# imironhead/ml_super_resolution

Measured on AMD Instinct MI355X. Metric: VDSR-20 training patches/sec (41x41, batch 256 per GPU); fwd HR megapixels/sec alongside, higher is better.
Workload: dtype f32; 1 GPU; BASELINE configs[2]: VDSR 20-layer 3x3x64 residual, RGB, batch 256x41x41 per GPU, fwd+bwd+TF-Adam, random-init weights; global_batch=256, patch=41, parallelism=dp1

## Files before the change

### ml_super_resolution_amd/csrc/conv_chain.hip

```cpp
#include "launchers.h"
namespace srx {

template <bool WT, int AUX>
__global__ __launch_bounds__(256, 1) void conv_chain_kernel(const ConvArgs a, const ChainPtrs c) {
    for (int l = 0; l < c.L; ++l) {
        ConvArgs al = a;
        al.x = c.x[l]; al.w = c.w[l]; al.bias = c.bias[l]; al.y = c.y[l];
        if (WT) al.mask = c.aux[l];
        else al.skip = c.aux[l];
        asm volatile("" : "+s"(al.N), "+s"(al.H), "+s"(al.W), "+s"(al.OH), "+s"(al.OW), "+s"(al.Cin), "+s"(al.Cout));
        asm volatile("" : "+s"(al.pad_t), "+s"(al.pad_l), "+s"(al.TH), "+s"(al.TW), "+s"(al.NTX), "+s"(al.RS));
        asm volatile("" : "+s"(al.units_total), "+s"(al.act), "+s"(al.post_relu), "+s"(al.mask_act), "+s"(al.buf_floats));
        conv_pipe_body<3, 3, 64, 4, WT, AUX, false>(al, l == 0);
        asm volatile("s_waitcnt vmcnt(0)" ::: "memory");
        __builtin_amdgcn_fence(__ATOMIC_RELEASE, "workgroup");
        __builtin_amdgcn_s_barrier();
        __builtin_amdgcn_fence(__ATOMIC_ACQUIRE, "workgroup");
    }
}

hipError_t launch_conv_chain(bool wt, bool aux, const ConvArgs& a, const ChainPtrs& c, int grid, size_t lds, hipStream_t s) {
    if (!wt) return aux ? hipErrorInvalidValue : launch_chain_with_lds(conv_chain_kernel<false, 0>, a, c, grid, lds, s);
    return aux ? launch_chain_with_lds(conv_chain_kernel<true, 1>, a, c, grid, lds, s)
               : launch_chain_with_lds(conv_chain_kernel<true, 0>, a, c, grid, lds, s);
}
}
```

### ml_super_resolution_amd/csrc/conv_kernels.hip.h

```cpp
#pragma once
#include <hip/hip_runtime.h>
#include <stdint.h>
#include <type_traits>

namespace srx {

typedef float f32x4 __attribute__((ext_vector_type(4)));

enum { ACT_NONE = 0, ACT_RELU = 1, ACT_TANH = 2, ACT_LRELU = 3, ACT_SIGMOID = 4 };

struct ConvArgs {
    const float* x;
    const float* w;
    const float* bias;
    const float* skip;
    const float* mask;
    float* y;
    int N, H, W, OH, OW, Cin, Cout;
    int pad_t, pad_l;
    int TH, TW, NTX, RS;
    int units_total;
    int act, post_relu, mask_act;
    float inv_rs;
    int stagger;
    int dbg;
    unsigned long long* trace;
    int buf_floats;
    int stride;
    int d2s_r, d2s_rc;
};

struct WgradArgs {
    const float* x;
    const float* dpre;
    float* part;
    int part_stride;
    int N, H, W, OH, OW, Cin, Cout;
    int pad_t, pad_l;
    int TH, TW, NTX, RS;
    int units_total;
    float inv_rs;
    int stagger;
    int zero_slot;
    int stride;
    unsigned long long* trace;
};

constexpr int kChainMax = 32;
struct ChainPtrs {
    const float* x[kChainMax];
    const float* w[kChainMax];
    const float* bias[kChainMax];
    const float* aux[kChainMax];
    float* y[kChainMax];
    int L;
};

template <int CINP>
struct Lds {
    static constexpr int PS = (CINP == 4) ? 4 : CINP + 4;
};

__device__ __forceinline__ float srx_tanhf(float x) {
    const float ax = fabsf(x);
    const float x2 = ax * ax;
    float p = fmaf(x2, -0.006274174898862839f, 0.021071631461381912f);
    p = fmaf(x2, p, -0.053852297365665436f);
    p = fmaf(x2, p, 0.13332585990428925f);
    p = fmaf(x2, p, -0.33333316445350647f);
    const float small = fmaf(x2 * ax, p, ax);
    const float e = __builtin_amdgcn_exp2f(ax * 2.8853900817779268f);
    const float big = fmaf(-2.0f, __builtin_amdgcn_rcpf(e + 1.0f), 1.0f);
    return copysignf(ax < 0.55f ? small : big, x);
}

typedef float f32x2 __attribute__((ext_vector_type(2)));
__device__ __forceinline__ f32x2 srx_tanhf2(f32x2 x) {
    const f32x2 ax = {fabsf(x[0]), fabsf(x[1])};
    const f32x2 x2 = ax * ax;
    f32x2 p = __builtin_elementwise_fma(x2, f32x2{-0.006274174898862839f, -0.006274174898862839f}, f32x2{0.021071631461381912f, 0.021071631461381912f});
    p = __builtin_elementwise_fma(x2, p, f32x2{-0.053852297365665436f, -0.053852297365665436f});
    p = __builtin_elementwise_fma(x2, p, f32x2{0.13332585990428925f, 0.13332585990428925f});
    p = __builtin_elementwise_fma(x2, p, f32x2{-0.33333316445350647f, -0.33333316445350647f});
    const f32x2 small = __builtin_elementwise_fma(x2 * ax, p, ax);
    const f32x2 t = ax * 2.8853900817779268f;
    f32x2 e = {__builtin_amdgcn_exp2f(t[0]), __builtin_amdgcn_exp2f(t[1])};
    e = e + 1.0f;
    const f32x2 r = {__builtin_amdgcn_rcpf(e[0]), __builtin_amdgcn_rcpf(e[1])};
// ... 319 lines not shown
#pragma unroll
            for (int tap = 0; tap < TAPS; ++tap)
#pragma unroll
                for (int j = 0; j < KSPT; ++j) {
                    const int soff = ((tap * a.Cin + 16 * (j / 4) + (j % 4)) * a.Cout) * 4;
                    wr[tap * KSPT + j] = __builtin_bit_cast(float, __builtin_amdgcn_raw_buffer_load_b32(rsrc, vlane, soff, 0));
                }
        } else {
            const int vlane = (co * a.Cin + 4 * kq) * 4;
#pragma unroll
            for (int tap = 0; tap < TAPS; ++tap)
#pragma unroll
                for (int g = 0; g < KSPT / 4; ++g) {
                    const int soff = (((TAPS - 1 - tap) * a.Cout) * a.Cin + 16 * g) * 4;
                    const f32x4 v = __builtin_bit_cast(f32x4, __builtin_amdgcn_raw_buffer_load_b128(rsrc, vlane, soff, 0));
#pragma unroll
                    for (int e = 0; e < 4; ++e) wr[tap * KSPT + 4 * g + e] = v[e];
                }
        }
        return;
    }
    const bool co_ok = co < a.Cout;
#pragma unroll
    for (int tap = 0; tap < TAPS; ++tap) {
#pragma unroll
        for (int j = 0; j < KSPT; ++j) {
            const int ci = (CINP >= 16) ? 16 * (j / 4) + 4 * kq + (j % 4) : kq;
            const bool ok = co_ok & (ci < a.Cin);
            const unsigned idx = !WT ? (unsigned)((tap * a.Cin + ci) * a.Cout + co)
                                     : (unsigned)(((TAPS - 1 - tap) * a.Cout + co) * a.Cin + ci);
            const float v = a.w[ok ? idx : 0u];
            wr[tap * KSPT + j] = ok ? v : 0.f;
        }
    }
}

template <int KH, int KW, int CINP, int G, bool GUARD, bool AUX>
__device__ __forceinline__ void conv_group(const float* lds, const float (&wr)[KH * KW * (CINP / 4)],
                                           const f32x4 bias4, const ConvArgs& a, int n, int h, int ow0,
                                           int th, int tw, float inv_tw, int m_first, int m_step, int n_active,
                                           int li, int kq, int cout0, unsigned long long& t_mfma, unsigned long long& t_pro,
                                           unsigned long long& t_epi) {
    constexpr int PS = Lds<CINP>::PS;
    constexpr int NG = (CINP >= 16) ? CINP / 16 : 1;
    const unsigned long long ts_pro = SRX_STAMP();
    const int npx = th * tw;
    const int cb = cout0 + 4 * kq;
    const bool vec = ((a.Cout & 3) == 0) && (cb + 3 < a.Cout) && !a.d2s_r;
    const size_t img_base = (size_t)n * a.OH * a.OW * a.Cout;
    int laddr[G];
    unsigned off[G];
    bool valid[G];
    f32x4 acc[G];
#pragma unroll
    for (int i = 0; i < G; ++i) {
        const int t = 16 * (m_first + i * m_step) + li;
        const bool live = (t < npx) & (i < n_active);
        valid[i] = live & (cb < a.Cout);
        const int tt = live ? t : 0;
        const int orow = fdiv_small(tt, inv_tw, tw);
        const int ocol = tt - orow * tw;
        laddr[i] = ((orow * a.RS + ocol) * PS << (a.stride - 1)) + ((CINP >= 16) ? 4 * kq : kq);
        off[i] = !valid[i] ? 0u
                 : (a.d2s_r ? (unsigned)(((h + orow) * a.d2s_r * a.OW + ow0 + ocol) * a.d2s_rc)
                            : (unsigned)(((h + orow) * a.OW + ow0 + ocol) * a.Cout + cb));
        acc[i] = bias4;
// ... 293 lines not shown
}

template <int CINP, int NB, bool Z = false, bool MID = false>
__device__ __forceinline__ void stage_tile_scalar(StageSeq& qi, StageSeq& qc, const StageGeo& G, __amdgpu_buffer_rsrc_t rsrc,
                                                  int voff_lane, int wl_lane) {
    constexpr int PPP = 256 / (CINP / 4);
    while (qi.left > 0) {
        f32x4 v[NB];
        unsigned long long mk[NB];
#pragma unroll
        for (int i = 0; i < NB; ++i) {
            unsigned long long t;
            int so;
            if constexpr (Z) {
                unsigned long long m;
                stage_mask_az<MID>(qi, G, m, t, mk[i]);
                stage_mask_bz(qi, m, t, mk[i], so);
                v[i] = stage_fire_z(m, mk[i], so, rsrc, voff_lane);
            } else {
                stage_mask_a(qi, G, mk[i], t);
                stage_mask_b(qi, mk[i], t, so);
                v[i] = stage_fire(mk[i], so, rsrc, voff_lane);
            }
            stage_next<PPP * CINP * 4>(qi, G.JP1, G.rowfix_g);
        }
#pragma unroll
        for (int i = 0; i < NB; ++i) {
            stage_commit((Z ? 2 : 1) * (NB - 1 - i), qc, mk[i], wl_lane, v[i]);
            stage_next<PPP * Lds<CINP>::PS * 4>(qc, G.JP1, G.rowfix_l);
        }
    }
}

#define SRX_PIN(x) asm volatile("" : "+v"(x))

template <int MAXG, int AUX>
struct PipePend {
    f32x4 acc[MAXG];
    f32x4 aux[(AUX == 1 || AUX == 2) ? MAXG : 1];
    __amdgpu_buffer_rsrc_t yrs;
    int m_first, gs;
};
struct PipeEpi {
    int lo, lo2;
    int cout4;
    int sh, rowb;
    int vo1, vo2, vo3;
};
template <int AUX>
__device__ __forceinline__ PipeEpi pipe_epi_setup(const ConvArgs& a) {
    PipeEpi e;
    e.lo = (a.act == ACT_RELU) ? 0 : (int)0x80000000;
    e.lo2 = (AUX == 2 && a.post_relu) ? 0 : (int)0x80000000;
    e.cout4 = (AUX == 4) ? 3 * a.d2s_r * 4 : a.Cout * 4;
    e.sh = (a.TW >= 32) ? 1 : 0;
    e.rowb = (AUX == 4) ? a.d2s_r * (a.OW * a.d2s_r * 3) * 4 : a.OW * a.Cout * 4;
    e.vo1 = e.vo2 = e.vo3 = 0;
    return e;
}
__device__ __forceinline__ f32x4 clamp_lo4(f32x4 v, int lo) {
#pragma unroll
    for (int e = 0; e < 4; ++e) {
        const float f = v[e];
        const int b = __float_as_int(f);
        v[e] = __int_as_float(b > lo ? b : lo);
    }
// ... 147 lines not shown
                for (int i = 2; i < nfr; ++i) frag(i);
                if (t < NST) {
                    if constexpr (Z) stg[t] = stage_fire_z(mv, mr, so, xrs, voff_lane);
                    else stg[t] = stage_fire(mk[t], so, xrs, voff_lane);
                }
                if (t >= NBLK / 2 && t < NBLK / 2 + NST) stage_next<PPP * PS * 4>(qc, SG.JP1, SG.rowfix_l);
            } else {
                if (t < NST) stage_next<PPP * CINP * 4>(qi, SG.JP1, SG.rowfix_g);
                if (t == A0) {
                    tcur += gs * TSTEP;
#pragma unroll
                    for (int i = 0; i < MAXG; ++i) lan[i] = *reinterpret_cast<const int*>(ldsb + tcur + i * TSTEP);
                }
            }
        }
#pragma unroll
        for (int i = 0; i < nfr; ++i) cg[i] = nxt[i];
    }
#pragma unroll
    for (int i = 0; i < MAXG; ++i) { cur[i] = cg[i]; la[i] = lan[i]; }
    if constexpr (G == 4)
        asm volatile("s_nop 15\n\ts_nop 7" : "+v"(acc[0]), "+v"(acc[1]), "+v"(acc[2]), "+v"(acc[3]));
    else
        asm volatile("s_nop 15\n\ts_nop 7" : "+v"(acc[0]), "+v"(acc[1]), "+v"(acc[2]));
#pragma unroll
    for (int i = 0; i < MAXG; ++i) {
        pd.acc[i] = (i < G) ? acc[i < G ? i : 0] : bias4;
        if (HASAUX) pd.aux[i] = (i < G) ? aux[i < G ? i : 0] : bias4;
    }
    pd.yrs = un.yrs; pd.m_first = m_first; pd.gs = gs;
    tt[1] += SRX_STAMP() - ts_m;
}

template <int KH, int KW, int CINP, int NCH, bool WT, int AUX, bool Z>
__device__ __forceinline__ void conv_pipe_body(const ConvArgs& a, bool lds_setup = true) {
    extern __shared__ __attribute__((aligned(16))) float lds[];
    constexpr int TAPS = KH * KW;
    constexpr int KSPT = CINP / 4;
    constexpr int NPART = 4 / NCH;
    constexpr int TPP = CINP / 4, PPP = 256 / TPP;
    constexpr int PS = Lds<CINP>::PS;
    constexpr int MAXG = 4;
    constexpr int TSTEP = 16 * PS * 4 * NPART;
    const int tid = threadIdx.x;
    const int lane = tid & 63;
    const int wave = __builtin_amdgcn_readfirstlane(tid >> 6);
    const int li = lane & 15, kq = lane >> 4;
    const int chunk = wave % NCH, part = wave / NCH;
    const int cout0 = chunk * 16;
    const int cb = cout0 + 4 * kq;
    const int c4 = tid % TPP, sp = tid / TPP;
    char* ldsb = reinterpret_cast<char*>(lds);

#ifdef SRX_TRACE
    const unsigned long long t_entry = __builtin_amdgcn_s_memtime(), rt_entry = __builtin_amdgcn_s_memrealtime();
#endif
    float wr[TAPS * KSPT];
    load_stationary_weights<TAPS, CINP, WT>(wr, a, cout0, li, kq);
    f32x4 bias4 = {0.f, 0.f, 0.f, 0.f};
    if (a.bias) {
#pragma unroll
        for (int e = 0; e < 4; ++e)
            if (cb + e < a.Cout) bias4[e] = a.bias[cb + e];
    }

    const long G_ = gridDim.x;
    const int u0 = (int)(((long)blockIdx.x * a.units_total) / G_);
    const int u1 = (int)(((long)(blockIdx.x + 1) * a.units_total) / G_);
    if (u0 >= u1) return;
    const int buf_bytes = a.buf_floats * 4;
    const int rows_full = a.TH + KH - 1;
    const int row_stride_b = a.RS * PS * 4;

    if (lds_setup) {
        const f32x4 z = {0.f, 0.f, 0.f, 0.f};
        for (int i = tid; !Z && i < (rows_full + 1) * a.pad_l * TPP; i += 256) {
            const int q = i / TPP, ch = i % TPP;
            const int r = q / a.pad_l, c = q % a.pad_l;
            const int off = ((r * a.RS + c) * PS + 4 * ch) * 4;
            if ((r * a.RS + c) * PS * 4 < buf_bytes) {
                *reinterpret_cast<f32x4*>(ldsb + off) = z;
                *reinterpret_cast<f32x4*>(ldsb + buf_bytes + off) = z;
            }
        }
        const int tw_ = Z ? a.TW : a.OW;
        const int n_sub_max = (a.TH * tw_ + 15) >> 4;
        for (int i = tid; i < n_sub_max * 64; i += 256) {
            const int m = i >> 6, L = i & 63;
            const int t = 16 * m + (L & 15);
            int addr = 0;
            if (t < a.TH * tw_) {
                const int orow = t / tw_, ocol = t - orow * tw_;
                addr = ((orow * a.RS + ocol) * PS + 4 * (L >> 4)) * 4;
            }
            const int where = ((16 * m + (L >> 2)) * PS + CINP + (L & 3)) * 4;
            *reinterpret_cast<int*>(ldsb + where) = addr;
// ... 29 lines not shown
        h = u % a.OH;
        n = u / a.OH;
        ow0 = 0;
        if constexpr (Z) {
            const int tx = n % a.NTX;
            n = n / a.NTX;
            ow0 = tx * a.TW;
            if (ow0 > a.OW - a.TW) ow0 = a.OW - a.TW;
        }
        th = a.TH;
        if (a.OH - h < th) th = a.OH - h;
        if (u1 - u < th) th = u1 - u;
    };
    auto stage_setup = [&](StageSeq& qi, StageSeq& qc, int h, int th, int ow0, int buf, bool active) {
        const int left = __builtin_amdgcn_readfirstlane(active ? (th + KH - 1) * JP : 0);
        qi.j = 0; qc.j = 0;
        qi.off = __builtin_amdgcn_readfirstlane(((h - a.pad_t) * a.W + ow0) * CINP * 4);
        if constexpr (Z) {
            SG.m_first = uniform64(__ballot(ow0 - a.pad_l + sp >= 0));
            const int c = (JP - 1) * PPP + sp;
            SG.m_last = uniform64(__ballot(c < a.RS && ow0 - a.pad_l + c < a.W));
        }
        qc.off = __builtin_amdgcn_readfirstlane(buf * buf_bytes);
        qi.left = left; qc.left = left;
        const int above = (a.pad_t > h) ? (a.pad_t - h) * JP : 0;
        qi.thr = __builtin_amdgcn_readfirstlane(left - above);
        qc.thr = 0;
    };

    unsigned long long tt[4] = {0, 0, 0, 0};
    int n, h, th, ow0;
    tile_of(u0, n, h, th, ow0);
    [[maybe_unused]] const unsigned long long t_begin = SRX_STAMP();
    __syncthreads();
    {
        StageSeq qi, qc;
        stage_setup(qi, qc, h, th, ow0, 0, true);
        const __amdgpu_buffer_rsrc_t xrs = __builtin_amdgcn_make_buffer_rsrc(
            const_cast<float*>(a.x) + ((size_t)n * a.H * a.W - a.pad_l) * CINP, 0, (a.H * a.W + a.pad_l) * CINP * 4, 0x00020000);
        stage_tile_scalar<CINP, 6, Z>(qi, qc, SG, xrs, voff_lane, wl_lane);
    }
    lds_barrier();
#pragma unroll
    for (int i = 0; i < TAPS * KSPT; ++i) {
        float t = wr[i];
        asm volatile("v_accvgpr_write_b32 %0, %1" : "=a"(wr[i]) : "v"(t));
    }
    [[maybe_unused]] const unsigned long long t_first = SRX_STAMP();

    PipePend<MAXG, AUX> pd;
#pragma unroll
    for (int i = 0; i < MAXG; ++i) pd.acc[i] = bias4;
    if (AUX == 1 || AUX == 2) {
#pragma unroll
        for (int i = 0; i < MAXG; ++i) pd.aux[i] = bias4;
    }
    pd.yrs = __builtin_amdgcn_make_buffer_rsrc(a.y, 0, 0, 0x00020000); pd.m_first = 0; pd.gs = 0;

    int cur_buf = 0;
    int u = u0;
    while (u < u1) {
        const unsigned long long ts_u = SRX_STAMP();
        tile_of(u, n, h, th, ow0);
        const int un_ = u + th;
        const bool has_next = un_ < u1;
        int n2 = n, h2 = h, th2 = th, ow2 = ow0;
        if (has_next) tile_of(un_, n2, h2, th2, ow2);
        StageSeq qi, qc;
        stage_setup(qi, qc, h2, th2, ow2, cur_buf ^ 1, has_next);
        const __amdgpu_buffer_rsrc_t xrs = __builtin_amdgcn_make_buffer_rsrc(
            const_cast<float*>(a.x) + ((size_t)n2 * a.H * a.W - a.pad_l) * CINP, 0, (a.H * a.W + a.pad_l) * CINP * 4, 0x00020000);

        PipeUnit un;
        const int npx = th * (Z ? a.TW : a.OW);
        const size_t unit_off = (AUX == 4) ? (((size_t)n * a.OH + h) * a.d2s_r * a.OW + ow0) * (size_t)(3 * a.d2s_r)
                                           : (((size_t)n * a.OH + h) * a.OW + ow0) * a.Cout;
        const int unit_bytes = (AUX == 4) ? ((th * a.d2s_r - 1) * a.OW + a.TW) * ep.cout4
                                          : (Z ? (th - 1) * a.OW + a.TW : npx) * ep.cout4;
        un.yrs = __builtin_amdgcn_make_buffer_rsrc(a.y + unit_off, 0, unit_bytes, 0x00020000);
        un.auxrs = __builtin_amdgcn_make_buffer_rsrc(const_cast<float*>((AUX == 1 || AUX == 2) ? auxp + unit_off : a.x), 0,
                                                     (AUX == 1 || AUX == 2) ? unit_bytes : 0, 0x00020000);

        const int n_sub = (npx + 15) >> 4;
        const int cnt = (n_sub - part + NPART - 1) / NPART;
        if (cnt > 0) {
            const int ng = (cnt + MAXG - 1) / MAXG;
            const int base = cnt / ng, rem = cnt % ng;
            int tcur = cur_buf * buf_bytes + tlane;
            int la[MAXG];
#pragma unroll
            for (int i = 0; i < MAXG; ++i) la[i] = *reinterpret_cast<const int*>(ldsb + tcur + i * TSTEP);
            f32x4 cur[MAXG];
#pragma unroll
            for (int i = 0; i < MAXG; ++i) cur[i] = *reinterpret_cast<const f32x4*>(ldsb + la[i]);
            tt[0] += SRX_STAMP() - ts_u;
            int idx = 0;
            for (int gi = 0; gi < ng; ++gi) {
                const int gs = base + (gi < rem ? 1 : 0);
                const int m_first = part + idx * NPART;
                if (gs == MAXG)
                    conv_group_pipe<KH, KW, CINP, MAXG, MAXG, AUX, NPART, Z>(ldsb, wr, bias4, row_stride_b, qi, qc, SG, xrs, voff_lane,
                                                                          wl_lane, la, cur, tcur, pd, un, m_first, gs, ep, vst, tt);
                else
                    conv_group_pipe<KH, KW, CINP, MAXG - 1, MAXG, AUX, NPART, Z>(ldsb, wr, bias4, row_stride_b, qi, qc, SG, xrs, voff_lane,
                                                                              wl_lane, la, cur, tcur, pd, un, m_first, gs, ep, vst, tt);
                idx += gs;
            }
        }
        const unsigned long long ts_d = SRX_STAMP();
        stage_tile_scalar<CINP, 6, Z>(qi, qc, SG, xrs, voff_lane, wl_lane);
        lds_barrier();
        tt[3] += SRX_STAMP() - ts_d;
        cur_buf ^= 1;
        u = un_;
    }
#pragma unroll
    for (int i = 0; i < MAXG; ++i) pipe_epilogue_one<MAXG, AUX, NPART, Z>(pd, i, ep, vst);
#ifdef SRX_TRACE
    if (a.trace && lane == 0) {
        unsigned long long* tr = a.trace + ((size_t)blockIdx.x * 4 + wave) * 12;
        tr[0] = t_begin; tr[1] = SRX_STAMP(); tr[2] = tt[1]; tr[3] = tt[3];
        tr[4] = __builtin_amdgcn_s_getreg((15 << 11) | (0 << 6) | 4);
        tr[5] = rt_entry; tr[6] = __builtin_amdgcn_s_memrealtime(); tr[7] = t_entry;
        tr[8] = t_first - t_begin; tr[9] = 0; tr[10] = tt[0]; tr[11] = tt[2];
    }
#endif
}

template <int KH, int KW, int CINP, int NCH, bool WT, int AUX>
__global__ __launch_bounds__(256, 1) void conv_pipe_kernel(const ConvArgs a) {
    conv_pipe_body<KH, KW, CINP, NCH, WT, AUX, false>(a);
}
template <int KH, int KW, int CINP, int NCH, bool WT, int AUX>
__global__ __launch_bounds__(256, 1) void conv_pipe_strip_kernel(const ConvArgs a) {
    static_assert(NCH == 4 || NCH == 2, "strip tiles: 64 or 32 output channels");
    static_assert(AUX != 4 || (!WT && NCH == 2), "sub-pixel store: forward, <= 32 output channels");
    conv_pipe_body<KH, KW, CINP, NCH, WT, AUX, true>(a);
}

template <int CINP, bool WT, int G>
__device__ __forceinline__ void conv_group_generic(const float* lds, const f32x4 bias4, const ConvArgs& a, int KH,
                                                   int KW, int n, int h, int ow0, int th, int tw, float inv_tw,
                                                   int m_first, int m_step, int li, int kq, int cout0) {
    constexpr int PS = Lds<CINP>::PS;
    constexpr int NG = (CINP >= 16) ? CINP / 16 : 1;
    const int TAPS = KH * KW;
    const int npx = th * tw;
    const int cb = cout0 + 4 * kq;
    const bool vec = ((a.Cout & 3) == 0) && (cb + 3 < a.Cout) && !a.d2s_r;
    const size_t img_base = (size_t)n * a.OH * a.OW * a.Cout;
    int laddr[G];
    unsigned off[G];
    bool valid[G];
    f32x4 acc[G];
#pragma unroll
    for (int i = 0; i < G; ++i) {
        const int t = 16 * (m_first + i * m_step) + li;
        valid[i] = (t < npx) & (cb < a.Cout);
        const int tt = (t < npx) ? t : 0;
        const int orow = fdiv_small(tt, inv_tw, tw);
        const int ocol = tt - orow * tw;
        laddr[i] = ((orow * a.RS + ocol) * PS << (a.stride - 1)) + ((CINP >= 16) ? 4 * kq : kq);
        off[i] = !valid[i] ? 0u
                 : (a.d2s_r ? (unsigned)(((h + orow) * a.d2s_r * a.OW + ow0 + ocol) * a.d2s_rc)
// ... 1497 lines not shown
```

### ml_super_resolution_amd/csrc/srx_api.hip

```cpp
#include <math.h>
#include <stdarg.h>
#include <atomic>
#include <stdio.h>
#include <stdlib.h>
#include <string.h>

#include "../../include/srx.h"
#include "elementwise.h"
#include "launchers.h"
#include "bf16x3.h"

using namespace srx;

namespace {

thread_local char g_err[512] = "";

struct Knobs {
    int pipe_default, narrow, wgrad_lin, wgrad_pipe, wgrad_pipe_strip, wgrad_rows_full, wgrad_1x1, wgrad_pack3, kwrows_min_pixels, big_route_min_pixels, strip_d2s, conv_1x1_min_pixels, pack3_dgrad;
    int chain, wgrad_batch;
    unsigned long long* trace;
    int dbg;
};
int env_int(const char* name, int dflt) { const char* e = getenv(name); return e ? atoi(e) : dflt; }
// ... 359 lines not shown
    a->inv_rs = 1.0f / (float)p.RS;
    a->stride = 1;
    a->stagger = stagger_sleeps(p);
    a->dbg = knobs().dbg;
    a->trace = knobs().trace;
}

int chain_plan(const srx_conv_desc* d, int op, int in_act, Plan* p, ConvArgs* a, int* grid) {
    int rc = check_desc(d);
    if (rc) return rc;
    if (op != SRX_OP_FWD && op != SRX_OP_BWD_DATA) return fail(SRX_ERR_BAD_ARG, "chain: op %d (forward or data gradient)", op);
    if (!use_chain()) return fail(SRX_ERR_UNSUPPORTED, "chain: switched off (srx_set_chain / SRX_CHAIN)");
    if (!use_pipe()) return fail(SRX_ERR_UNSUPPORTED, "chain: conv path 0");
    if (!launch_conv_chain) return fail(SRX_ERR_UNSUPPORTED, "chain: this build has no chain kernels");
    if (d->precision != SRX_PRECISION_FP32) return fail(SRX_ERR_UNSUPPORTED, "chain: precision %d (exact fp32 only)", d->precision);
    if (d->KH != 3 || d->KW != 3 || d->Cin != 64 || d->Cout != 64 || d->stride != 1 || d->pad_mode != SRX_PAD_SAME)
        return fail(SRX_ERR_UNSUPPORTED, "chain: only 3x3 64->64 stride-1 SAME layers");
    if (d->subpixel_r > 1 || d->post_add_relu) return fail(SRX_ERR_UNSUPPORTED, "chain: no sub-pixel store or post-add activation");
    if (op == SRX_OP_FWD && d->act != SRX_ACT_NONE && d->act != SRX_ACT_RELU)
        return fail(SRX_ERR_UNSUPPORTED, "chain: forward activation %d (none / ReLU)", d->act);
    if (op == SRX_OP_BWD_DATA && in_act != SRX_ACT_NONE && in_act != SRX_ACT_RELU)
        return fail(SRX_ERR_UNSUPPORTED, "chain: in_act %d (none / ReLU)", in_act);
    int pt, pl, OH, OW;
    geometry(d, &pt, &pl, &OH, &OW);
    rc = (op == SRX_OP_FWD) ? make_plan(d->N, d->H, d->W, OH, OW, d->Cin, d->Cout, 3, 3, pt, pl, p, true)
                            : make_plan(d->N, OH, OW, d->H, d->W, d->Cout, d->Cin, 3, 3, 2 - pt, 2 - pl, p);
    if (rc) return rc;
    memset(a, 0, sizeof(*a));
    if (op == SRX_OP_FWD) fill_conv_args(a, *p, d->N, d->H, d->W, d->Cin, d->Cout);
    else fill_conv_args(a, *p, d->N, OH, OW, d->Cout, d->Cin);
    a->act = (op == SRX_OP_FWD) ? d->act : SRX_ACT_NONE;
    a->post_relu = 0;
    a->mask_act = (op == SRX_OP_FWD) ? 0 : in_act;
    a->trace = nullptr;
    const int ppp = 256 / (p->cinp / 4);
    const bool pipe_ok = p->cinp == 64 && p->nch == 4 && p->NTX == 1 && p->RS >= ppp && p->RS == a->W + a->pad_l && 16 <= a->OW &&
                         (long)a->H * a->W * a->Cin * 4 < (1L << 31) - 64 && (long)a->OH * a->OW * a->Cout * 4 < (1L << 31) - 64;
    if (!pipe_ok) return fail(SRX_ERR_UNSUPPORTED, "chain: the shape is not on the full-width pipelined route (column strips?)");
    *grid = p->grid < pipe_grid() ? p->grid : pipe_grid();
    if (d->N % *grid) return fail(SRX_ERR_UNSUPPORTED, "chain: N %d is not a multiple of the grid %d (a workgroup would split an image)", d->N, *grid);
    a->buf_floats = (int)(p->lds_bytes / 4);
    return SRX_OK;
}

}

extern "C" {

int srx_set_chain(int on) {
    const int old = g_chain.exchange(on < 0 ? -1 : (on ? 1 : 0), std::memory_order_relaxed);
    return old < 0 ? (knobs().chain ? 1 : 0) : old;
}

int srx_conv_chain_supported(const srx_conv_desc* d, int op, int in_act) {
    Plan p;
    ConvArgs a;
    int grid;
    return chain_plan(d, op, in_act, &p, &a, &grid) == SRX_OK ? 1 : 0;
}

int srx_conv_chain(const srx_conv_desc* d, int op, int in_act, int layers, const float* const* x, const float* const* w,
                   const float* const* bias, const float* const* aux, float* const* y, srx_stream_t stream) {
    if (layers < 1 || layers > kChainMax) return fail(SRX_ERR_BAD_ARG, "chain: %d layers (1..%d)", layers, kChainMax);
    if (!x || !w || !y) return fail(SRX_ERR_BAD_ARG, "null pointer array");
    Plan p;
    ConvArgs a;
    int grid;
// ... 718 lines not shown
```

Measured before the change: 19450 patches/s.

## Prefetch next layer's input tile and weights across chained conv layers

In the persistent conv-chain kernel, each layer's last iteration now stages the first input tile of the next layer into LDS, but only when that tile's rows were already written by this block long enough ago. It also loads the next layer's stationary weights and bias into a carried register struct before the epilogue, so the inter-layer gap no longer pays a cold tile stage and weight load. The cost is extra register pressure from the carried 144-float weight array, plus a correctness risk: the prefetched input depends on block-local row ordering, and other blocks' writes to those rows may not yet be visible.

```diff
diff --git a/ml_super_resolution_amd/csrc/conv_chain.hip b/ml_super_resolution_amd/csrc/conv_chain.hip
--- a/ml_super_resolution_amd/csrc/conv_chain.hip
+++ b/ml_super_resolution_amd/csrc/conv_chain.hip
@@ -3,6 +3,17 @@
 
 template <bool WT, int AUX>
 __global__ __launch_bounds__(256, 1) void conv_chain_kernel(const ConvArgs a, const ChainPtrs c) {
+    ChainLink<9 * 16> lk;
+    lk.c = &c; lk.staged = false; lk.cur_buf = 0;
+    {
+        const int lane = threadIdx.x & 63, wave = __builtin_amdgcn_readfirstlane(threadIdx.x >> 6);
+        ConvArgs a0 = a;
+        a0.w = c.w[0]; a0.bias = c.bias[0];
+        load_stationary_weights<9, 64, WT>(lk.wr, a0, wave * 16, lane & 15, lane >> 4);
+        const f32x4 z = {0.f, 0.f, 0.f, 0.f};
+        lk.bias4 = z;
+        load_bias4(lk.bias4, a0, wave * 16 + 4 * (lane >> 4));
+    }
     for (int l = 0; l < c.L; ++l) {
         ConvArgs al = a;
         al.x = c.x[l]; al.w = c.w[l]; al.bias = c.bias[l]; al.y = c.y[l];
@@ -11,7 +22,8 @@
         asm volatile("" : "+s"(al.N), "+s"(al.H), "+s"(al.W), "+s"(al.OH), "+s"(al.OW), "+s"(al.Cin), "+s"(al.Cout));
         asm volatile("" : "+s"(al.pad_t), "+s"(al.pad_l), "+s"(al.TH), "+s"(al.TW), "+s"(al.NTX), "+s"(al.RS));
         asm volatile("" : "+s"(al.units_total), "+s"(al.act), "+s"(al.post_relu), "+s"(al.mask_act), "+s"(al.buf_floats));
-        conv_pipe_body<3, 3, 64, 4, WT, AUX, false>(al, l == 0);
+        lk.l = l;
+        conv_pipe_body<3, 3, 64, 4, WT, AUX, false, true>(al, l == 0, &lk);
         asm volatile("s_waitcnt vmcnt(0)" ::: "memory");
         __builtin_amdgcn_fence(__ATOMIC_RELEASE, "workgroup");
         __builtin_amdgcn_s_barrier();
diff --git a/ml_super_resolution_amd/csrc/conv_kernels.hip.h b/ml_super_resolution_amd/csrc/conv_kernels.hip.h
--- a/ml_super_resolution_amd/csrc/conv_kernels.hip.h
+++ b/ml_super_resolution_amd/csrc/conv_kernels.hip.h
@@ -439,6 +439,13 @@
             const float v = a.w[ok ? idx : 0u];
             wr[tap * KSPT + j] = ok ? v : 0.f;
         }
+    }
+}
+__device__ __forceinline__ void load_bias4(f32x4& bias4, const ConvArgs& a, int cb) {
+    if (a.bias) {
+#pragma unroll
+        for (int e = 0; e < 4; ++e)
+            if (cb + e < a.Cout) bias4[e] = a.bias[cb + e];
     }
 }
 
@@ -1011,8 +1018,18 @@
     tt[1] += SRX_STAMP() - ts_m;
 }
 
-template <int KH, int KW, int CINP, int NCH, bool WT, int AUX, bool Z>
-__device__ __forceinline__ void conv_pipe_body(const ConvArgs& a, bool lds_setup = true) {
+template <int NW>
+struct ChainLink {
+    const ChainPtrs* c;
+    int l;
+    bool staged;
+    int cur_buf;
+    float wr[NW];
+    f32x4 bias4;
+};
+template <int KH, int KW, int CINP, int NCH, bool WT, int AUX, bool Z, bool CHAIN = false>
+__device__ __forceinline__ void conv_pipe_body(const ConvArgs& a, bool lds_setup = true,
+                                               ChainLink<KH * KW * (CINP / 4)>* lk = nullptr) {
     extern __shared__ __attribute__((aligned(16))) float lds[];
     constexpr int TAPS = KH * KW;
     constexpr int KSPT = CINP / 4;
@@ -1035,12 +1052,14 @@
     const unsigned long long t_entry = __builtin_amdgcn_s_memtime(), rt_entry = __builtin_amdgcn_s_memrealtime();
 #endif
     float wr[TAPS * KSPT];
-    load_stationary_weights<TAPS, CINP, WT>(wr, a, cout0, li, kq);
     f32x4 bias4 = {0.f, 0.f, 0.f, 0.f};
-    if (a.bias) {
-#pragma unroll
-        for (int e = 0; e < 4; ++e)
-            if (cb + e < a.Cout) bias4[e] = a.bias[cb + e];
+    if constexpr (CHAIN) {
+#pragma unroll
+        for (int i = 0; i < TAPS * KSPT; ++i) wr[i] = lk->wr[i];
+        bias4 = lk->bias4;
+    } else {
+        load_stationary_weights<TAPS, CINP, WT>(wr, a, cout0, li, kq);
+        load_bias4(bias4, a, cb);
     }
 
     const long G_ = gridDim.x;
@@ -1136,15 +1155,23 @@
     int n, h, th, ow0;
     tile_of(u0, n, h, th, ow0);
     [[maybe_unused]] const unsigned long long t_begin = SRX_STAMP();
-    __syncthreads();
-    {
-        StageSeq qi, qc;
-        stage_setup(qi, qc, h, th, ow0, 0, true);
-        const __amdgpu_buffer_rsrc_t xrs = __builtin_amdgcn_make_buffer_rsrc(
-            const_cast<float*>(a.x) + ((size_t)n * a.H * a.W - a.pad_l) * CINP, 0, (a.H * a.W + a.pad_l) * CINP * 4, 0x00020000);
-        stage_tile_scalar<CINP, 6, Z>(qi, qc, SG, xrs, voff_lane, wl_lane);
-    }
-    lds_barrier();
+    int cur_buf = 0;
+    bool first_here = true;
+    if constexpr (CHAIN) {
+        first_here = !lk->staged;
+        if (!first_here) cur_buf = lk->cur_buf;
+    }
+    if (first_here) {
+        __syncthreads();
+        {
+            StageSeq qi, qc;
+            stage_setup(qi, qc, h, th, ow0, 0, true);
+            const __amdgpu_buffer_rsrc_t xrs = __builtin_amdgcn_make_buffer_rsrc(
+                const_cast<float*>(a.x) + ((size_t)n * a.H * a.W - a.pad_l) * CINP, 0, (a.H * a.W + a.pad_l) * CINP * 4, 0x00020000);
+            stage_tile_scalar<CINP, 6, Z>(qi, qc, SG, xrs, voff_lane, wl_lane);
+        }
+        lds_barrier();
+    }
 #pragma unroll
     for (int i = 0; i < TAPS * KSPT; ++i) {
         float t = wr[i];
@@ -1161,8 +1188,9 @@
     }
     pd.yrs = __builtin_amdgcn_make_buffer_rsrc(a.y, 0, 0, 0x00020000); pd.m_first = 0; pd.gs = 0;
 
-    int cur_buf = 0;
     int u = u0;
+    [[maybe_unused]] int u_prev = u0;
+    [[maybe_unused]] bool pre = false;
     while (u < u1) {
         const unsigned long long ts_u = SRX_STAMP();
         tile_of(u, n, h, th, ow0);
@@ -1170,10 +1198,20 @@
         const bool has_next = un_ < u1;
         int n2 = n, h2 = h, th2 = th, ow2 = ow0;
         if (has_next) tile_of(un_, n2, h2, th2, ow2);
+        const float* xsrc = a.x;
+        if constexpr (CHAIN) {
+            const int rows_need = (a.TH < a.OH - 1) ? a.TH : a.OH - 1;
+            pre = !has_next && lk->l + 1 < lk->c->L && u0 + rows_need < u_prev;
+            if (pre) {
+                tile_of(u0, n2, h2, th2, ow2);
+                xsrc = lk->c->x[lk->l + 1];
+            }
+            u_prev = u;
+        }
         StageSeq qi, qc;
-        stage_setup(qi, qc, h2, th2, ow2, cur_buf ^ 1, has_next);
+        stage_setup(qi, qc, h2, th2, ow2, cur_buf ^ 1, CHAIN ? (has_next || pre) : has_next);
         const __amdgpu_buffer_rsrc_t xrs = __builtin_amdgcn_make_buffer_rsrc(
-            const_cast<float*>(a.x) + ((size_t)n2 * a.H * a.W - a.pad_l) * CINP, 0, (a.H * a.W + a.pad_l) * CINP * 4, 0x00020000);
+            const_cast<float*>(xsrc) + ((size_t)n2 * a.H * a.W - a.pad_l) * CINP, 0, (a.H * a.W + a.pad_l) * CINP * 4, 0x00020000);
 
         PipeUnit un;
         const int npx = th * (Z ? a.TW : a.OW);
@@ -1217,6 +1255,19 @@
         tt[3] += SRX_STAMP() - ts_d;
         cur_buf ^= 1;
         u = un_;
+    }
+    if constexpr (CHAIN) {
+        lk->staged = pre;
+        lk->cur_buf = cur_buf;
+        if (lk->l + 1 < lk->c->L) {
+            ConvArgs an = a;
+            an.w = lk->c->w[lk->l + 1];
+            an.bias = lk->c->bias[lk->l + 1];
+            load_stationary_weights<TAPS, CINP, WT>(lk->wr, an, cout0, li, kq);
+            const f32x4 z = {0.f, 0.f, 0.f, 0.f};
+            lk->bias4 = z;
+            load_bias4(lk->bias4, an, cb);
+        }
     }
 #pragma unroll
     for (int i = 0; i < MAXG; ++i) pipe_epilogue_one<MAXG, AUX, NPART, Z>(pd, i, ep, vst);
```

Result: no change. 19450 patches/s (-0.0%).

## Prefetch next layer's first input tile during last tile of chained conv

Applied to the files above, without the earlier changes.

Inside the persistent multi-layer conv chain kernel, the last tile iteration of each layer now stages the first input tile of the next layer into the spare LDS buffer. The next layer then skips its cold staging step and its barrier, which hides per-layer startup latency. This only turns on when each workgroup owns whole images and handles at least four tiles, so that the halo rows it prefetches come from its own already-stored output. It adds an extra barrier with a full memory wait in the last tile and depends on careful ordering of the deferred stores.

```diff
diff --git a/ml_super_resolution_amd/csrc/chain_prefetch.h b/ml_super_resolution_amd/csrc/chain_prefetch.h
--- /dev/null
+++ b/ml_super_resolution_amd/csrc/chain_prefetch.h
@@ -0,0 +1,12 @@
+#pragma once
+namespace srx {
+
+constexpr int chain_tiles_per_workgroup(int rows, int OH, int TH) {
+    return (OH > 0 && TH > 0) ? (rows / OH) * ((OH + TH - 1) / TH) : 0;
+}
+
+constexpr bool chain_prefetch_ok(int rows, int OH, int TH) {
+    return OH > 0 && rows >= OH && rows % OH == 0 && chain_tiles_per_workgroup(rows, OH, TH) >= 4;
+}
+
+}
diff --git a/ml_super_resolution_amd/csrc/conv_chain.hip b/ml_super_resolution_amd/csrc/conv_chain.hip
--- a/ml_super_resolution_amd/csrc/conv_chain.hip
+++ b/ml_super_resolution_amd/csrc/conv_chain.hip
@@ -1,8 +1,12 @@
 #include "launchers.h"
+#include "chain_prefetch.h"
 namespace srx {
 
 template <bool WT, int AUX>
 __global__ __launch_bounds__(256, 1) void conv_chain_kernel(const ConvArgs a, const ChainPtrs c) {
+    const bool prefetch = chain_prefetch_ok(a.units_total / (int)gridDim.x, a.OH, a.TH);
+    ChainLink lk;
+    lk.buf = -1;
     for (int l = 0; l < c.L; ++l) {
         ConvArgs al = a;
         al.x = c.x[l]; al.w = c.w[l]; al.bias = c.bias[l]; al.y = c.y[l];
@@ -11,7 +15,8 @@
         asm volatile("" : "+s"(al.N), "+s"(al.H), "+s"(al.W), "+s"(al.OH), "+s"(al.OW), "+s"(al.Cin), "+s"(al.Cout));
         asm volatile("" : "+s"(al.pad_t), "+s"(al.pad_l), "+s"(al.TH), "+s"(al.TW), "+s"(al.NTX), "+s"(al.RS));
         asm volatile("" : "+s"(al.units_total), "+s"(al.act), "+s"(al.post_relu), "+s"(al.mask_act), "+s"(al.buf_floats));
-        conv_pipe_body<3, 3, 64, 4, WT, AUX, false>(al, l == 0);
+        lk.next_x = (prefetch && l + 1 < c.L) ? c.x[l + 1] : nullptr;
+        conv_pipe_body<3, 3, 64, 4, WT, AUX, false, true>(al, l == 0, &lk);
         asm volatile("s_waitcnt vmcnt(0)" ::: "memory");
         __builtin_amdgcn_fence(__ATOMIC_RELEASE, "workgroup");
         __builtin_amdgcn_s_barrier();
diff --git a/ml_super_resolution_amd/csrc/conv_kernels.hip.h b/ml_super_resolution_amd/csrc/conv_kernels.hip.h
--- a/ml_super_resolution_amd/csrc/conv_kernels.hip.h
+++ b/ml_super_resolution_amd/csrc/conv_kernels.hip.h
@@ -54,6 +54,10 @@
     const float* aux[kChainMax];
     float* y[kChainMax];
     int L;
+};
+struct ChainLink {
+    const float* next_x;
+    int buf;
 };
 
 template <int CINP>
@@ -1011,8 +1015,8 @@
     tt[1] += SRX_STAMP() - ts_m;
 }
 
-template <int KH, int KW, int CINP, int NCH, bool WT, int AUX, bool Z>
-__device__ __forceinline__ void conv_pipe_body(const ConvArgs& a, bool lds_setup = true) {
+template <int KH, int KW, int CINP, int NCH, bool WT, int AUX, bool Z, bool LINK = false>
+__device__ __forceinline__ void conv_pipe_body(const ConvArgs& a, bool lds_setup = true, ChainLink* lk = nullptr) {
     extern __shared__ __attribute__((aligned(16))) float lds[];
     constexpr int TAPS = KH * KW;
     constexpr int KSPT = CINP / 4;
@@ -1136,15 +1140,20 @@
     int n, h, th, ow0;
     tile_of(u0, n, h, th, ow0);
     [[maybe_unused]] const unsigned long long t_begin = SRX_STAMP();
-    __syncthreads();
-    {
-        StageSeq qi, qc;
-        stage_setup(qi, qc, h, th, ow0, 0, true);
-        const __amdgpu_buffer_rsrc_t xrs = __builtin_amdgcn_make_buffer_rsrc(
-            const_cast<float*>(a.x) + ((size_t)n * a.H * a.W - a.pad_l) * CINP, 0, (a.H * a.W + a.pad_l) * CINP * 4, 0x00020000);
-        stage_tile_scalar<CINP, 6, Z>(qi, qc, SG, xrs, voff_lane, wl_lane);
-    }
-    lds_barrier();
+    int cur_buf = 0;
+    if (LINK && lk->buf >= 0) {
+        cur_buf = lk->buf;
+    } else {
+        __syncthreads();
+        {
+            StageSeq qi, qc;
+            stage_setup(qi, qc, h, th, ow0, 0, true);
+            const __amdgpu_buffer_rsrc_t xrs = __builtin_amdgcn_make_buffer_rsrc(
+                const_cast<float*>(a.x) + ((size_t)n * a.H * a.W - a.pad_l) * CINP, 0, (a.H * a.W + a.pad_l) * CINP * 4, 0x00020000);
+            stage_tile_scalar<CINP, 6, Z>(qi, qc, SG, xrs, voff_lane, wl_lane);
+        }
+        lds_barrier();
+    }
 #pragma unroll
     for (int i = 0; i < TAPS * KSPT; ++i) {
         float t = wr[i];
@@ -1161,19 +1170,27 @@
     }
     pd.yrs = __builtin_amdgcn_make_buffer_rsrc(a.y, 0, 0, 0x00020000); pd.m_first = 0; pd.gs = 0;
 
-    int cur_buf = 0;
     int u = u0;
     while (u < u1) {
         const unsigned long long ts_u = SRX_STAMP();
         tile_of(u, n, h, th, ow0);
         const int un_ = u + th;
         const bool has_next = un_ < u1;
+        const bool link = LINK && !has_next && lk->next_x != nullptr;
         int n2 = n, h2 = h, th2 = th, ow2 = ow0;
         if (has_next) tile_of(un_, n2, h2, th2, ow2);
+        else if (link) tile_of(u0, n2, h2, th2, ow2);
+        if (link) {
+            asm volatile("s_waitcnt vmcnt(0)" ::: "memory");
+            __builtin_amdgcn_fence(__ATOMIC_RELEASE, "workgroup");
+            __builtin_amdgcn_s_barrier();
+            __builtin_amdgcn_fence(__ATOMIC_ACQUIRE, "workgroup");
+        }
         StageSeq qi, qc;
-        stage_setup(qi, qc, h2, th2, ow2, cur_buf ^ 1, has_next);
+        stage_setup(qi, qc, h2, th2, ow2, cur_buf ^ 1, has_next || link);
+        const float* xsrc = link ? lk->next_x : a.x;
         const __amdgpu_buffer_rsrc_t xrs = __builtin_amdgcn_make_buffer_rsrc(
-            const_cast<float*>(a.x) + ((size_t)n2 * a.H * a.W - a.pad_l) * CINP, 0, (a.H * a.W + a.pad_l) * CINP * 4, 0x00020000);
+            const_cast<float*>(xsrc) + ((size_t)n2 * a.H * a.W - a.pad_l) * CINP, 0, (a.H * a.W + a.pad_l) * CINP * 4, 0x00020000);
 
         PipeUnit un;
         const int npx = th * (Z ? a.TW : a.OW);
@@ -1217,6 +1234,7 @@
         tt[3] += SRX_STAMP() - ts_d;
         cur_buf ^= 1;
         u = un_;
+        if (LINK) lk->buf = link ? cur_buf : -1;
     }
 #pragma unroll
     for (int i = 0; i < MAXG; ++i) pipe_epilogue_one<MAXG, AUX, NPART, Z>(pd, i, ep, vst);
```

Result: no change. 19460 patches/s before, 19450 patches/s after (-0.1%).

## Add specialized ENT path for 3x3x64 pipelined conv entry and tile stepping

Applied to the files above, without the earlier changes.

Adds a specialized variant of the pipelined conv body for 3x3 64-channel full-width tiles. Stationary weights are loaded straight into AGPRs with buffer loads, which removes the VGPR-to-AGPR copy. The first tile is staged with a deeper batch of 21 in-flight loads. Next-tile coordinates are computed incrementally instead of through tile_of, the per-tile LDS address reads are hoisted to one read before the loop, and the integer division in the group split is replaced by a closed form. The aim is to cut kernel entry latency and per-tile scalar and LDS overhead, in exchange for more register pressure and a new route whose correctness rests on tiles being contiguous full-width rows.

```diff
diff --git a/ml_super_resolution_amd/csrc/conv_chain.hip b/ml_super_resolution_amd/csrc/conv_chain.hip
--- a/ml_super_resolution_amd/csrc/conv_chain.hip
+++ b/ml_super_resolution_amd/csrc/conv_chain.hip
@@ -11,7 +11,10 @@
         asm volatile("" : "+s"(al.N), "+s"(al.H), "+s"(al.W), "+s"(al.OH), "+s"(al.OW), "+s"(al.Cin), "+s"(al.Cout));
         asm volatile("" : "+s"(al.pad_t), "+s"(al.pad_l), "+s"(al.TH), "+s"(al.TW), "+s"(al.NTX), "+s"(al.RS));
         asm volatile("" : "+s"(al.units_total), "+s"(al.act), "+s"(al.post_relu), "+s"(al.mask_act), "+s"(al.buf_floats));
-        conv_pipe_body<3, 3, 64, 4, WT, AUX, false>(al, l == 0);
+#ifdef SRX_TRACE
+        if (al.trace) al.trace += (size_t)l * gridDim.x * 4 * 12;
+#endif
+        conv_pipe_body<3, 3, 64, 4, WT, AUX, false, true>(al, l == 0);
         asm volatile("s_waitcnt vmcnt(0)" ::: "memory");
         __builtin_amdgcn_fence(__ATOMIC_RELEASE, "workgroup");
         __builtin_amdgcn_s_barrier();
diff --git a/ml_super_resolution_amd/csrc/conv_kernels.hip.h b/ml_super_resolution_amd/csrc/conv_kernels.hip.h
--- a/ml_super_resolution_amd/csrc/conv_kernels.hip.h
+++ b/ml_super_resolution_amd/csrc/conv_kernels.hip.h
@@ -439,6 +439,39 @@
             const float v = a.w[ok ? idx : 0u];
             wr[tap * KSPT + j] = ok ? v : 0.f;
         }
+    }
+}
+template <int TAPS, int CINP, bool WT>
+__device__ __forceinline__ void load_stationary_weights_acc(float (&wr)[TAPS * (CINP / 4)], const ConvArgs& a, int cout0,
+                                                            int li, int kq) {
+    constexpr int KSPT = CINP / 4;
+    static_assert(CINP >= 16, "exact-fit 16-channel groups");
+    constexpr int oob = 0x7fffffff;
+    const int co = cout0 + li;
+    __amdgpu_buffer_rsrc_t rsrc =
+        __builtin_amdgcn_make_buffer_rsrc(const_cast<float*>(a.w), 0, TAPS * a.Cin * a.Cout * 4, 0x00020000);
+    if (!WT) {
+        const int vlane = (co < a.Cout) ? (4 * kq * a.Cout + co) * 4 : oob;
+#pragma unroll
+        for (int tap = 0; tap < TAPS; ++tap)
+#pragma unroll
+            for (int j = 0; j < KSPT; ++j) {
+                const int soff = ((tap * a.Cin + 16 * (j / 4) + (j % 4)) * a.Cout) * 4;
+                asm volatile("buffer_load_dword %0, %1, %2, %3 offen"
+                             : "=a"(wr[tap * KSPT + j]) : "v"(vlane), "s"(rsrc), "s"(soff) : "memory");
+            }
+    } else {
+        const int vlane = (co < a.Cout) ? (co * a.Cin + 4 * kq) * 4 : oob;
+#pragma unroll
+        for (int tap = 0; tap < TAPS; ++tap)
+#pragma unroll
+            for (int g = 0; g < KSPT / 4; ++g) {
+                const int soff = (((TAPS - 1 - tap) * a.Cout) * a.Cin + 16 * g) * 4;
+                f32x4 v;
+                asm volatile("buffer_load_dwordx4 %0, %1, %2, %3 offen" : "=a"(v) : "v"(vlane), "s"(rsrc), "s"(soff) : "memory");
+#pragma unroll
+                for (int e = 0; e < 4; ++e) wr[tap * KSPT + 4 * g + e] = v[e];
+            }
     }
 }
 
@@ -798,6 +831,29 @@
     }
 }
 
+template <int CINP, int NB>
+__device__ __forceinline__ void stage_tile_deep(StageSeq& qi, StageSeq& qc, const StageGeo& G, __amdgpu_buffer_rsrc_t rsrc,
+                                                int voff_lane, int wl_lane) {
+    constexpr int PPP = 256 / (CINP / 4);
+    while (qi.left > 0) {
+        f32x4 v[NB];
+#pragma unroll
+        for (int i = 0; i < NB; ++i) {
+            unsigned long long m, t;
+            int so;
+            stage_mask_a(qi, G, m, t);
+            stage_mask_b(qi, m, t, so);
+            v[i] = stage_fire(m, so, rsrc, voff_lane);
+            stage_next<PPP * CINP * 4>(qi, G.JP1, G.rowfix_g);
+        }
+#pragma unroll
+        for (int i = 0; i < NB; ++i) {
+            stage_commit(NB - 1 - i, qc, stage_mask_full(qc, G), wl_lane, v[i]);
+            stage_next<PPP * Lds<CINP>::PS * 4>(qc, G.JP1, G.rowfix_l);
+        }
+    }
+}
+
 #define SRX_PIN(x) asm volatile("" : "+v"(x))
 
 template <int MAXG, int AUX>
@@ -1011,8 +1067,9 @@
     tt[1] += SRX_STAMP() - ts_m;
 }
 
-template <int KH, int KW, int CINP, int NCH, bool WT, int AUX, bool Z>
+template <int KH, int KW, int CINP, int NCH, bool WT, int AUX, bool Z, bool ENT = false>
 __device__ __forceinline__ void conv_pipe_body(const ConvArgs& a, bool lds_setup = true) {
+    static_assert(!ENT || !Z, "ENT: full-width tiles only");
     extern __shared__ __attribute__((aligned(16))) float lds[];
     constexpr int TAPS = KH * KW;
     constexpr int KSPT = CINP / 4;
@@ -1035,7 +1092,8 @@
     const unsigned long long t_entry = __builtin_amdgcn_s_memtime(), rt_entry = __builtin_amdgcn_s_memrealtime();
 #endif
     float wr[TAPS * KSPT];
-    load_stationary_weights<TAPS, CINP, WT>(wr, a, cout0, li, kq);
+    if constexpr (ENT) load_stationary_weights_acc<TAPS, CINP, WT>(wr, a, cout0, li, kq);
+    else load_stationary_weights<TAPS, CINP, WT>(wr, a, cout0, li, kq);
     f32x4 bias4 = {0.f, 0.f, 0.f, 0.f};
     if (a.bias) {
 #pragma unroll
@@ -1137,18 +1195,30 @@
     tile_of(u0, n, h, th, ow0);
     [[maybe_unused]] const unsigned long long t_begin = SRX_STAMP();
     __syncthreads();
+    [[maybe_unused]] int la0[MAXG];
+    if constexpr (ENT) {
+#pragma unroll
+        for (int i = 0; i < MAXG; ++i) la0[i] = *reinterpret_cast<const int*>(ldsb + tlane + i * TSTEP);
+    }
     {
         StageSeq qi, qc;
         stage_setup(qi, qc, h, th, ow0, 0, true);
         const __amdgpu_buffer_rsrc_t xrs = __builtin_amdgcn_make_buffer_rsrc(
             const_cast<float*>(a.x) + ((size_t)n * a.H * a.W - a.pad_l) * CINP, 0, (a.H * a.W + a.pad_l) * CINP * 4, 0x00020000);
-        stage_tile_scalar<CINP, 6, Z>(qi, qc, SG, xrs, voff_lane, wl_lane);
+        if constexpr (ENT) {
+            stage_tile_deep<CINP, 21>(qi, qc, SG, xrs, voff_lane, wl_lane);
+            asm volatile("s_waitcnt vmcnt(0)" ::: "memory");
+        } else {
+            stage_tile_scalar<CINP, 6, Z>(qi, qc, SG, xrs, voff_lane, wl_lane);
+        }
     }
     lds_barrier();
-#pragma unroll
-    for (int i = 0; i < TAPS * KSPT; ++i) {
-        float t = wr[i];
-        asm volatile("v_accvgpr_write_b32 %0, %1" : "=a"(wr[i]) : "v"(t));
+    if constexpr (!ENT) {
+#pragma unroll
+        for (int i = 0; i < TAPS * KSPT; ++i) {
+            float t = wr[i];
+            asm volatile("v_accvgpr_write_b32 %0, %1" : "=a"(wr[i]) : "v"(t));
+        }
     }
     [[maybe_unused]] const unsigned long long t_first = SRX_STAMP();
 
@@ -1165,11 +1235,22 @@
     int u = u0;
     while (u < u1) {
         const unsigned long long ts_u = SRX_STAMP();
-        tile_of(u, n, h, th, ow0);
+        if constexpr (!ENT) tile_of(u, n, h, th, ow0);
         const int un_ = u + th;
         const bool has_next = un_ < u1;
         int n2 = n, h2 = h, th2 = th, ow2 = ow0;
-        if (has_next) tile_of(un_, n2, h2, th2, ow2);
+        if constexpr (ENT) {
+            if (has_next) {
+                h2 = h + th;
+                if (h2 >= a.OH) { h2 = 0; n2 = n + 1; }
+                th2 = a.TH;
+                if (a.OH - h2 < th2) th2 = a.OH - h2;
+                asm volatile("" : "+s"(th2));
+                if (u1 - un_ < th2) th2 = u1 - un_;
+            }
+        } else if (has_next) {
+            tile_of(un_, n2, h2, th2, ow2);
+        }
         StageSeq qi, qc;
         stage_setup(qi, qc, h2, th2, ow2, cur_buf ^ 1, has_next);
         const __amdgpu_buffer_rsrc_t xrs = __builtin_amdgcn_make_buffer_rsrc(
@@ -1189,11 +1270,23 @@
         const int cnt = (n_sub - part + NPART - 1) / NPART;
         if (cnt > 0) {
             const int ng = (cnt + MAXG - 1) / MAXG;
-            const int base = cnt / ng, rem = cnt % ng;
+            int base, rem;
+            if constexpr (ENT) {
+                static_assert(MAXG == 4, "ceil(d / ng) below is written out for d <= 3");
+                const int d = MAXG * ng - cnt;
+                const int miss = (d == 0) ? 0 : (ng >= d) ? 1 : (ng == 1) ? d : 2;
+                base = MAXG - miss;
+                rem = cnt - base * ng;
+            } else {
+                base = cnt / ng; rem = cnt % ng;
+            }
             int tcur = cur_buf * buf_bytes + tlane;
             int la[MAXG];
 #pragma unroll
-            for (int i = 0; i < MAXG; ++i) la[i] = *reinterpret_cast<const int*>(ldsb + tcur + i * TSTEP);
+            for (int i = 0; i < MAXG; ++i) {
+                if constexpr (ENT) la[i] = la0[i] + cur_buf * buf_bytes;
+                else la[i] = *reinterpret_cast<const int*>(ldsb + tcur + i * TSTEP);
+            }
             f32x4 cur[MAXG];
 #pragma unroll
             for (int i = 0; i < MAXG; ++i) cur[i] = *reinterpret_cast<const f32x4*>(ldsb + la[i]);
@@ -1217,6 +1310,7 @@
         tt[3] += SRX_STAMP() - ts_d;
         cur_buf ^= 1;
         u = un_;
+        if constexpr (ENT) { n = n2; h = h2; th = th2; }
     }
 #pragma unroll
     for (int i = 0; i < MAXG; ++i) pipe_epilogue_one<MAXG, AUX, NPART, Z>(pd, i, ep, vst);
@@ -1233,7 +1327,7 @@
 
 template <int KH, int KW, int CINP, int NCH, bool WT, int AUX>
 __global__ __launch_bounds__(256, 1) void conv_pipe_kernel(const ConvArgs a) {
-    conv_pipe_body<KH, KW, CINP, NCH, WT, AUX, false>(a);
+    conv_pipe_body<KH, KW, CINP, NCH, WT, AUX, false, KH == 3 && KW == 3 && CINP == 64 && NCH == 4>(a);
 }
 template <int KH, int KW, int CINP, int NCH, bool WT, int AUX>
 __global__ __launch_bounds__(256, 1) void conv_pipe_strip_kernel(const ConvArgs a) {
diff --git a/ml_super_resolution_amd/csrc/srx_api.hip b/ml_super_resolution_amd/csrc/srx_api.hip
--- a/ml_super_resolution_amd/csrc/srx_api.hip
+++ b/ml_super_resolution_amd/csrc/srx_api.hip
@@ -415,7 +415,6 @@
     a->act = (op == SRX_OP_FWD) ? d->act : SRX_ACT_NONE;
     a->post_relu = 0;
     a->mask_act = (op == SRX_OP_FWD) ? 0 : in_act;
-    a->trace = nullptr;
     const int ppp = 256 / (p->cinp / 4);
     const bool pipe_ok = p->cinp == 64 && p->nch == 4 && p->NTX == 1 && p->RS >= ppp && p->RS == a->W + a->pad_l && 16 <= a->OW &&
                          (long)a->H * a->W * a->Cin * 4 < (1L << 31) - 64 && (long)a->OH * a->OW * a->Cout * 4 < (1L << 31) - 64;
```

Result: no change. 19490 patches/s before, 19560 patches/s after (median of 6 runs) (+0.4%).
